# OpenDriveLab/Vista

Hardware: AMD Instinct MI355X
Metric: denoise steps/sec, 25-frame 576x1024 latent, 50-step EDM @ 1/2/4/8 GPU (higher is better)
Workload: dtype bf16; 1 GPU; 1xMI355X single GPU: 25x576x1024 (latent 25x4x72x128), 50-step EulerEDM, VanillaCFG 2.5 (N=50 images per UNet call), bf16, random-init 1.65B VideoUNet, synthetic latents; frames=25, cfg_images_per_call=50, sampler=EulerEDM s_churn=0, 50-step schedule, parallelism=single GPU

## Files before the change

include/vista_hip.h:

```cpp
#ifndef VISTA_HIP_H
#define VISTA_HIP_H
#include <stdint.h>
#ifdef __cplusplus
extern "C" {
#endif

enum { VK_AMODE_DENSE = 0, VK_AMODE_CONV3X3 = 1, VK_AMODE_TEMPORAL3 = 2, VK_AMODE_CONV3D = 3 };
enum { VK_EPI_LINEAR = 0, VK_EPI_GEGLU = 1, VK_EPI_TRANS = 2 };

typedef struct VkGemmDesc {
    const void* A;
    const void* Wt;
    void* out;
    const float* bias;
    const float* rowvec;
    const void* res1;
    const void* res2;
    int32_t M, N, K;
    int32_t lda, ldc, ld_res1, ld_res2, ldv, rows_per_vec;
    float alpha, beta;
    int32_t amode, epi, out_f32;
    int32_t H, Wd, Cin, Hout, Wout, stride, ups;
    int32_t T, S;
    int32_t tile_cfg;
// ... 205 lines not shown
```

vista_amd/csrc/gemm.hip:

```cpp
#include <stdlib.h>

#include "common.h"
#include "vista_hip.h"

#include "gemm_common.h"

extern "C" int vk_gemm_pipe_fit(const VkGemmDesc* d);
extern "C" int vk_gemm_pipe_launch(const VkGemmDesc* d, void* stream, int ksplit);
extern "C" int vk_gemm_pipe_gnstat_ok(const VkGemmDesc* d, int ksplit);
extern "C" int vk_gemm_pipe2_fit(const VkGemmDesc* d);
extern "C" int vk_gemm_pipe2_launch(const VkGemmDesc* d, void* stream);
extern "C" int vk_gemm_stream_fit(const VkGemmDesc* d);
extern "C" int vk_gemm_stream_launch(const VkGemmDesc* d, void* stream);

namespace {

constexpr int TILE5_MAX_K_DEFAULT = 320;

__device__ uint4 g_zero16;

template <int AMODE, int EPI, bool OUT_F32, int WM, int WN, int FM, int FN>
__global__ __launch_bounds__(WM * WN * 64, (WM * WN == 16) ? 4 : 2) void gemm_kernel(const VkGemmDesc p, const int ksplit) {
    constexpr int BM = WM * FM * 32, BN = WN * FN * 32;
    constexpr int NT = WM * WN * 64;
// ... 410 lines not shown
    if (full == 0 || rem == 0 || rem * 100 > (long long)max_pct * 256) return 0;
    const long long tm_main = full * 256 / tilesN;
    if (tm_main <= 0 || tm_main >= tilesM) return 0;
    const int m_split = d->m_begin + (int)tm_main * 256;
    const long long small = (long long)((d->m_end - m_split + 127) / 128) * (d->N / 160);
    if (small > 512) return 0;
    return m_split;
}

inline bool pipe2_wanted(const VkGemmDesc* d, const TileChoice& t, bool gnstat) {
    if (!(d->tile_cfg & 16) || gnstat || t.ksplit != 1 || d->amode != AMODE_DENSE || d->out_f32) return false;
    if (d->epi == EPI_LINEAR && t.cfg != 4 && t.cfg != 5 && t.cfg != 7) return false;
    return vk_gemm_pipe2_fit(d) != 0;
}

enum GemmFamily { FAM_STREAM, FAM_PIPE2, FAM_PIPE, FAM_TILED };
struct GemmPlan {
    int family;
    int cfg;
    int ksplit;
    int tail_row;
    int rowstat_slabs;
    int gnstat_slots;
};

GemmPlan plan_gemm(VkGemmDesc& d, bool rowstat, bool gnstat) {
    static const bool stream_on = [] { const char* e = getenv("VISTA_GEMM_STREAM"); return !e || atoi(e) != 0; }();
    const int force = d.tile_cfg & 7;
    if (d.m_begin == 0 && d.m_end == d.M && !(d.tile_cfg & 16) && (force == 6 || (stream_on && !rowstat))) {
        if (const int fit = vk_gemm_stream_fit(&d)) return {FAM_STREAM, 6, 1, 0, d.N / (32 * fit), 0};
    }
    if (force == 6) d.tile_cfg &= ~7;
    const TileChoice t = choose_tile(&d, rowstat, gnstat);
    GemmPlan p{FAM_TILED, t.cfg, t.ksplit, 0, 0, 0};
    if (pipe2_wanted(&d, t, gnstat)) p.family = FAM_PIPE2;
    else if (t.cfg == 7) p.family = FAM_PIPE;
    if (p.family == FAM_PIPE) p.tail_row = tail_split_row(&d, t);
    int bn, wn;
    tile_geometry(t.cfg, bn, wn);
    p.rowstat_slabs = ((d.N + bn - 1) / bn) * wn;
    if (p.family == FAM_PIPE && p.ksplit == 1 && p.tail_row == 0 && !rowstat && vk_gemm_pipe_gnstat_ok(&d, 1)) p.gnstat_slots = d.M / 64;
    return p;
}
// ... 41 lines not shown
    if (p.family == FAM_PIPE2) return vk_gemm_pipe2_launch(d, stream);
    if (p.family == FAM_PIPE && p.tail_row) {
        VkGemmDesc head = *d, tail = *d;
        head.m_end = p.tail_row;
        tail.m_begin = p.tail_row;
        rc = vk_gemm_pipe_launch(&head, stream, 1);
        return rc != VK_OK ? rc : launch_tiled(&tail, stream, 5, 1);
    }
    rc = (p.family == FAM_PIPE) ? vk_gemm_pipe_launch(d, stream, p.ksplit) : launch_tiled(d, stream, p.cfg, p.ksplit);
    if (rc != VK_OK || p.ksplit == 1) return rc;
    return launch_splitk_finish(d, stream, p.ksplit);
}

inline int validate(const VkGemmDesc* d) {
    if (!d || !d->A || !d->Wt || !d->out) return VK_EINVAL;
    if (d->M <= 0 || d->N <= 0 || d->K <= 0 || (d->K % BK) != 0 || (d->N % 4) != 0 || d->tile_cfg < 0 || (d->tile_cfg & ~(64 | 16)) > 7) return VK_EINVAL;
    if (d->m_begin < 0 || d->m_end < 0 || d->m_end > d->M || (d->m_end != 0 && d->m_begin >= d->m_end) || (d->m_end == 0 && d->m_begin >= d->M)) return VK_EINVAL;
    if ((d->m_begin != 0 || (d->m_end != 0 && d->m_end != d->M)) && d->epi == EPI_TRANS) return VK_EINVAL;
    if (d->amode != AMODE_DENSE && (d->Cin <= 0 || (d->Cin % BK) != 0)) return VK_EINVAL;
    if (d->amode == AMODE_DENSE && (d->lda % 8) != 0) return VK_EINVAL;
    if (d->amode == AMODE_CONV3X3 && (d->K != 9 * d->Cin || d->stride < 1 || d->stride > 2 || d->ups < 1 || d->ups > 2)) return VK_EINVAL;
    if (d->amode == AMODE_TEMPORAL3 && (d->K != 3 * d->Cin || d->T <= 0 || d->S <= 0)) return VK_EINVAL;
    if (d->amode == AMODE_CONV3D && (d->K != 27 * d->Cin || d->T <= 0 || d->H <= 0 || d->Wd <= 0 || d->H >= 4096 || d->Wd >= 4096 ||
                                     (long long)d->M != (long long)(d->M / (d->H * d->Wd)) * d->H * d->Wd)) return VK_EINVAL;
    if ((d->rowvec || d->rowvec2) && d->rows_per_vec <= 0) return VK_EINVAL;
    if (d->rowvec2 && (!d->res2 || d->epi != EPI_LINEAR)) return VK_EINVAL;
    if (d->A2 && (d->amode != AMODE_DENSE || d->k_split <= 0 || d->k_split >= d->K || (d->k_split % BK) != 0 || (d->lda2 % 8) != 0)) return VK_EINVAL;
    if (d->ln_stats && (d->amode != AMODE_DENSE || d->A2 || !d->ln_colsum || d->ln_parts <= 0 || d->ln_parts > 64 || !(d->ln_eps > 0.f))) return VK_EINVAL;
    if (d->rowstat_out && (d->epi != EPI_LINEAR || d->out_f32)) return VK_EINVAL;
    if (d->act != 0 && (d->act != 1 || d->epi != EPI_LINEAR)) return VK_EINVAL;
    if (d->mx8_out && (!d->mx8_scales || d->epi != EPI_LINEAR || d->out_f32 || (d->N % 320) != 0 || d->mx8_cols <= 0 || (d->mx8_cols % 320) != 0 ||
                       d->mx8_cols > d->N || (d->ld_mx8 % 16) != 0 || d->ld_mx8 < d->mx8_cols || d->ld_mx8s * 32 < d->mx8_cols ||
                       (((size_t)d->mx8_out) & 15) != 0 || d->rowstat_out || (d->ldc % 8) != 0 || (((size_t)d->out) & 15) != 0 ||
                       (d->amode != AMODE_DENSE) || d->res1 || d->res2 || d->rowvec || d->rowvec2 ||
                       (unsigned long long)d->M * 2ull * (unsigned)d->ldc >= 0xfffff000ull))
        return VK_EINVAL;
    if (d->alt_cols_from != 0 && (d->alt_cols_from < 0 || (d->alt_cols_from % 32) != 0 || d->alt_cols_from >= d->N || d->epi != EPI_LINEAR || d->out_f32 ||
                                  d->rowstat_out || d->gnstat_out || d->mx8_out))
        return VK_EINVAL;
    return VK_OK;
}

int plan_for(const VkGemmDesc* d, VkGemmDesc& q, bool rowstat, bool gnstat, GemmPlan& p) {
    const int rc = validate(d);
    if (rc != VK_OK) return rc;
    q = *d;
    norm_row_range(q);
    p = plan_gemm(q, rowstat || q.rowstat_out != nullptr, gnstat || q.gnstat_out != nullptr);
    return VK_OK;
}

}

extern "C" int vk_gemm_rowstat_parts(const VkGemmDesc* d) {
    VkGemmDesc q;
    GemmPlan p;
    const int rc = plan_for(d, q, true, false, p);
    if (rc != VK_OK) return rc;
    return (q.epi != EPI_LINEAR || q.out_f32) ? VK_EINVAL : p.rowstat_slabs;
}

extern "C" int vk_gemm_tile_choice(const VkGemmDesc* d) {
    VkGemmDesc q;
    GemmPlan p;
// ... 27 lines not shown
```

vista_amd/csrc/gemm_common.h:

```cpp
#pragma once
#include "common.h"
#include "vista_hip.h"

namespace {

enum { AMODE_DENSE = 0, AMODE_CONV3X3 = 1, AMODE_TEMPORAL3 = 2, AMODE_CONV3D = 3 };
enum { EPI_LINEAR = 0, EPI_GEGLU = 1, EPI_TRANS = 2 };

constexpr int BK = 64;

inline bool norm_row_range(VkGemmDesc& d) {
    if (d.m_end == 0) d.m_end = d.M;
    return d.m_begin >= 0 && d.m_begin < d.m_end && d.m_end <= d.M;
}


__device__ __forceinline__ uint4 widen_pair(uint2 qa, uint2 qb) {
    const auto rx = __builtin_amdgcn_permlane32_swap(qa.x, qb.x, false, false);
    const auto ry = __builtin_amdgcn_permlane32_swap(qa.y, qb.y, false, false);
    return make_uint4(rx[0], ry[0], rx[1], ry[1]);
}

#ifndef VK_EPI_NT_STORES
#define VK_EPI_NT_STORES 0
// ... 392 lines not shown
        const int c0 = 32 * fi + 8 * g + 2 * h;
        const int G0 = c0 / CPG, G1 = (c0 + 4) / CPG;
        if (G0 == G1) {
            gs[G0] = vk_dot2(w, one, gs[G0]);
            gq[G0] = vk_dot2(w, w, gq[G0]);
        } else {
            const uint32_t v0 = w & lo_mask, v1 = w & ~lo_mask;
            gs[G0] = vk_dot2(v0, one, gs[G0]);
            gq[G0] = vk_dot2(v0, v0, gq[G0]);
            gs[G1] = vk_dot2(v1, one, gs[G1]);
            gq[G1] = vk_dot2(v1, v1, gq[G1]);
        }
    }
}

template <int NRES, bool LN, bool MX, int FX, int FY, int FM, int FN, int BN, int CAP, int GNC = 0>
__device__ __forceinline__ void epilogue_linear_lds_body(const VkGemmDesc& p, f32x16_t (&acc)[FX][FY], int m0, int n0, int wm, int wn, int l31, int lh,
                                                         int stat_part, const float2* lnrow, const float* ev, int img0) {
    constexpr int MW = FM * 32, NW = FN * 32, U = FX * FY;
    constexpr int GN_NG = GNC ? NW / GNC : 1;
    constexpr int ROOM = (CAP - 16 * U - 36) / 8;
    constexpr int DA = NRES == 0 ? 0 : ((ROOM / NRES < 1 ? 1 : ROOM / NRES) < U ? (ROOM / NRES < 1 ? 1 : ROOM / NRES) : U);
    constexpr bool mx_tile = MX;
    const bool a_is_r1 = p.res1 != nullptr;
    const uint16_t* __restrict__ ra = (const uint16_t*)(a_is_r1 ? p.res1 : p.res2);
    const uint16_t* __restrict__ rb = (const uint16_t*)p.res2;
    const int lda_ = a_is_r1 ? p.ld_res1 : p.ld_res2;
    const int c0 = wn * NW + 4 * lh;
    const int wide_off = n0 + wn * NW + 8 * lh;
    bool row_ok[FY];
    int mrow[FY];
    uint32_t rao[FY], rbo[FY], oo[FY];
    char* const outb = (char*)p.out;
#pragma unroll
    for (int fj = 0; fj < FY; ++fj) {
        const int m = m0 + wm * MW + fj * 32 + l31;
        row_ok[fj] = m < p.m_end;
        mrow[fj] = row_ok[fj] ? m : p.m_end - 1;
        if (NRES >= 1) rao[fj] = ((uint32_t)mrow[fj] * (uint32_t)lda_ + (uint32_t)wide_off) * 2u;
        if (NRES == 2) rbo[fj] = ((uint32_t)mrow[fj] * (uint32_t)p.ld_res2 + (uint32_t)wide_off) * 2u;
        oo[fj] = ((uint32_t)mrow[fj] * (uint32_t)p.ldc + (uint32_t)(wide_off - (p.mx8_out ? p.mx8_cols : 0))) * 2u;
    }
    static_assert(GNC == 0 || (MW % 64 == 0 && NW == 160 && NW % GNC == 0 && !MX), "gnstat_out: wave tiles of 64-row blocks x 160 columns of whole channel groups");
    float gs[GN_NG], gq[GN_NG];
    if constexpr (GNC != 0) {
#pragma unroll
        for (int i = 0; i < GN_NG; ++i) { gs[i] = 0.f; gq[i] = 0.f; }
    }
    const uint32_t gn_lo_mask = lh ? 0u : 0xffffffffu;
    uint4 wa[U][2], wb[U][2];
    auto issue = [&](int fj, int fi, int u) {
        if (NRES >= 1) { wa[u][0] = *(const uint4*)((const char*)ra + rao[fj] + fi * 64); wa[u][1] = *(const uint4*)((const char*)ra + rao[fj] + fi * 64 + 32); }
        if (NRES == 2) { wb[u][0] = *(const uint4*)((const char*)rb + rbo[fj] + fi * 64); wb[u][1] = *(const uint4*)((const char*)rb + rbo[fj] + fi * 64 + 32); }
    };
#pragma unroll
// ... 84 lines not shown
        if constexpr (GNC != 0 && FY > 2) {
            if ((fj & 1) == 1) {
                const int mb = m0 + wm * MW + (fj >> 1) * 64;
                gn_reduce_store<GN_NG>(gs, gq, (float*)p.gnstat_out + (size_t)(mb >> 6) * 64, (n0 + wn * NW) / GNC, l31 | (lh << 5), mb < p.m_end);
#pragma unroll
                for (int i = 0; i < GN_NG; ++i) { gs[i] = 0.f; gq[i] = 0.f; }
            }
        }
    }
    if constexpr (GNC != 0 && FY == 2) {
        const int mb = m0 + wm * MW;
        gn_reduce_store<GN_NG>(gs, gq, (float*)p.gnstat_out + (size_t)(mb >> 6) * 64, (n0 + wn * NW) / GNC, l31 | (lh << 5), mb < p.m_end);
    }
}

template <int FX, int FY, int FM, int FN, int BN, int CAP = 128, int GN_CPG = 0, int GN_NRES = 0>
__device__ __forceinline__ void gemm_epilogue_linear_lds(const VkGemmDesc& p, f32x16_t (&acc)[FX][FY], int m0, int n0, int wm, int wn, int l31, int lh,
                                                         int stat_part, const float2* lnrow, const float* ev, int img0) {
    if constexpr (GN_CPG != 0) {
        epilogue_linear_lds_body<GN_NRES, false, false, FX, FY, FM, FN, BN, CAP, GN_CPG>(p, acc, m0, n0, wm, wn, l31, lh, stat_part, nullptr, ev, img0);
        return;
    }
    const int nres = (p.res1 != nullptr) + (p.res2 != nullptr);
    if constexpr (BN == 320) {
        if (p.mx8_out != nullptr && n0 < p.mx8_cols) {
            if (lnrow != nullptr) epilogue_linear_lds_body<0, true, true, FX, FY, FM, FN, BN, CAP>(p, acc, m0, n0, wm, wn, l31, lh, stat_part, lnrow, ev, img0);
            else epilogue_linear_lds_body<0, false, true, FX, FY, FM, FN, BN, CAP>(p, acc, m0, n0, wm, wn, l31, lh, stat_part, lnrow, ev, img0);
            return;
        }
    }
#define VK_EPI_BODY(NR, LNF) epilogue_linear_lds_body<NR, LNF, false, FX, FY, FM, FN, BN, CAP>(p, acc, m0, n0, wm, wn, l31, lh, stat_part, lnrow, ev, img0)
    if (lnrow != nullptr) {
        if (nres == 0) VK_EPI_BODY(0, true);
// ... 56 lines not shown
```

vista_amd/csrc/gemm_pipe.hip:

```cpp
#include "common.h"
#include "vista_hip.h"

#include "gemm_common.h"

namespace {

constexpr int PBM = 256, PBN = 320, PNT = 512;
constexpr int PFX = 5, PFY = 2;
constexpr int PRPP = PNT / 8;
constexpr int PAP = PBM / PRPP, PWP = PBN / PRPP;
constexpr int PA_BYTES = PBM * 128, PSTAGE = (PBM + PBN) * 128;
constexpr int PCAP = 256;
constexpr int APAR0 = 6 * PAP;
typedef unsigned amask_t;
constexpr unsigned P_OOB = 0xffffff00u;
constexpr unsigned long long P_LIMIT = 0xfffff000ull;
static_assert(PAP + PWP <= PFX * PFY && 8 * PAP <= 32, "the piece schedule issues one piece after each MFMA of the first k-substep");

typedef __attribute__((address_space(3))) void* lptr_t;

#define PIPE_MMA(FI, X, Y, C) C = vk_mfma(X, Y, C)

#define PIPE_SB() __builtin_amdgcn_sched_barrier(0)

template <int AMODE, int EPI, bool NT_A, bool SPLIT, int GN_CPG = 0, int GN_NRES = 0, bool PF = false>
__global__ __launch_bounds__(PNT, 2) void gemm_pipe_kernel(const VkGemmDesc p, const int ksplit) {
    static_assert(!PF || AMODE == AMODE_DENSE, "the L2 prefetch is written for the dense loader");
    constexpr int LN_OFF = 2 * PSTAGE, EV_OFF = LN_OFF + PBM * 8;
    constexpr int NTAPS = (AMODE == AMODE_CONV3X3) ? 9 : (AMODE == AMODE_TEMPORAL3) ? 3 : 1;
    constexpr bool WALK = (EPI == EPI_GEGLU);
    __shared__ __attribute__((aligned(16))) char smem[2 * PSTAGE + PBM * 8 + epi_vec_floats(PBN) * 4];
#ifdef PIPE_TIMING
    unsigned long long tm_k0, tm_dma = 0, tm_bar = 0, tm_loop = 0, tm_epi = 0, tm_ksteps = 0;
    asm volatile("s_memtime %0\n s_waitcnt lgkmcnt(0)" : "=s"(tm_k0) :: "memory");
#endif

    const int tilesN = p.N / PBN;
    const int tilesM = (p.m_end - p.m_begin + PBM - 1) / PBM;
    const int ntiles = tilesM * tilesN;
    const int tid = threadIdx.x;
    const int lane = tid & 63, wave = tid >> 6;
    const int wm = wave >> 1, wn = wave & 1;
    const int l31 = lane & 31, lh = lane >> 5;
    int kslice = 0;
    auto tile_of = [&](const int bid, int& tm, int& tn) __attribute__((always_inline)) {
        int logical = xcd_remap(bid, SPLIT ? ntiles * ksplit : ntiles);
        if (SPLIT) { kslice = logical / ntiles; logical -= kslice * ntiles; }
        if (tilesN < 8 || (long long)p.N * p.K * 2 <= (3LL << 20)) {
            tn = logical % tilesN;
            tm = logical / tilesN;
        } else {
            constexpr int GM = 8;
            const int panel = logical / (GM * tilesN), r = logical - panel * (GM * tilesN);
            const int gm = (tilesM - panel * GM < GM) ? tilesM - panel * GM : GM;
            tm = panel * GM + r % gm;
            tn = r / gm;
        }
        if constexpr (AMODE == AMODE_TEMPORAL3) {
            if (p.tile_cfg & 8) return;
            const int nblk = p.S / PBM;
            if (nblk * PBM == p.S && p.m_begin == 0 && tilesM == (p.M / p.S) * nblk && (long long)p.S * p.Cin * 2 > (3LL << 20)) {
                const int per_clip = p.T * nblk, clip = tm / per_clip, r = tm - clip * per_clip;
// ... 2 lines not shown
            }
        }
    };

    const int lc = tid & 7, lr = tid >> 3;
    const int lsrc = lc ^ ((lr >> 1) & 7);
    const int wave_u = __builtin_amdgcn_readfirstlane(wave);
    const unsigned voff_w = ((unsigned)lr * (unsigned)p.K + (unsigned)lsrc * 8u) * 2u;
    const unsigned wpass = (unsigned)PRPP * (unsigned)p.K * 2u;
    const unsigned apass = (unsigned)PRPP * (unsigned)(AMODE == AMODE_DENSE ? p.lda : p.Cin) * 2u;

    __amdgpu_buffer_rsrc_t rw, ra;
    unsigned voff_a[PAP];
    amask_t amask = 0;
    auto setup = [&](const int m0, const int n0) __attribute__((always_inline)) {
        rw = __builtin_amdgcn_make_buffer_rsrc((void*)((const uint16_t*)p.Wt + (size_t)n0 * p.K), 0, (int)((unsigned)PBN * (unsigned)p.K * 2u), 0x00020000);
        amask = 0;
        if (AMODE == AMODE_DENSE) {
            const int rows = (p.m_end - m0 < PBM) ? p.m_end - m0 : PBM;
            ra = __builtin_amdgcn_make_buffer_rsrc((void*)((const uint16_t*)p.A + (size_t)m0 * p.lda), 0,
                                                   (int)(((unsigned)(rows - 1) * (unsigned)p.lda + (unsigned)p.K) * 2u), 0x00020000);
            voff_a[0] = ((unsigned)lr * (unsigned)p.lda + (unsigned)lsrc * 8u) * 2u;
        } else if (AMODE == AMODE_CONV3X3) {
            const int hw = p.Hout * p.Wout;
            ra = __builtin_amdgcn_make_buffer_rsrc((void*)p.A, 0, (int)((unsigned)(p.M / hw) * (unsigned)(p.H * p.Wd) * (unsigned)p.Cin * 2u), 0x00020000);
#pragma unroll
            for (int i = 0; i < PAP; ++i) {
                const int m = m0 + lr + PRPP * i;
                const int img = m / hw;
                const int rem = m - img * hw;
                const int oy = rem / p.Wout, ox = rem - oy * p.Wout;
                const int y0 = oy * p.stride - (p.asym_pad ? 0 : 1), x0 = ox * p.stride - (p.asym_pad ? 0 : 1);
                const int sh = p.ups - 1;
// ... 37 lines not shown
            const unsigned v = voff_a[0] + (unsigned)j * apass;
            if (NT_A) __builtin_amdgcn_raw_ptr_buffer_load_lds(ra, dst, 16, v, (unsigned)kb, 0, 2);
            else __builtin_amdgcn_raw_ptr_buffer_load_lds(ra, dst, 16, v, (unsigned)kb, 0, 0);
        } else if (AMODE == AMODE_CONV3X3) {
            const int ky = tap / 3, kx = tap - ky * 3;
            const bool ok = ((amask >> (6 * j + ky)) & (amask >> (6 * j + 3 + kx)) & 1u) != 0;
            unsigned v;
            if (p.ups == 2) {
                const unsigned dy = ((unsigned)((amask >> (APAR0 + 2 * j)) & 1u) + (unsigned)(ky + 1)) >> 1, dx = ((unsigned)((amask >> (APAR0 + 1 + 2 * j)) & 1u) + (unsigned)(kx + 1)) >> 1;
                v = voff_a[j] + (dy * (unsigned)p.Wd + dx) * ((unsigned)p.Cin * 2u);
            } else {
                v = voff_a[j] + (unsigned)((ky * p.Wd + kx) * p.Cin) * 2u;
            }
            if (!ok) v = P_OOB;
            __builtin_amdgcn_raw_ptr_buffer_load_lds(ra, dst, 16, v, (unsigned)c0b, 0, 0);
        } else {
            const unsigned tapoff = (unsigned)((tap - 1) * p.S * p.Cin) * 2u;
            const bool ok = ((amask >> (3 * j + tap)) & 1u) != 0;
            const unsigned v = ok ? voff_a[0] + (unsigned)j * apass + tapoff : P_OOB;
            __builtin_amdgcn_raw_ptr_buffer_load_lds(ra, dst, 16, v, (unsigned)c0b, 0, 0);
        }
    };
    auto dma_next = [&]() __attribute__((always_inline)) {
        kb += BK * 2;
        if (AMODE != AMODE_DENSE) {
            if (++tap == NTAPS) { tap = 0; c0b += BK * 2; }
        }
    };
    auto dma_q = [&](const int q, const int stage) __attribute__((always_inline)) { dma_piece(q < PAP ? PWP + q : q - PAP, stage); };

// ... 165 lines not shown

        int te = tid;
        asm volatile("" : "+v"(te));
        const int e_wave = te >> 6, e_l31 = te & 31, e_lh = (te >> 5) & 1;
        const int e_wm = e_wave >> 1, e_wn = e_wave & 1;
        const float2* const lnp = p.ln_stats != nullptr ? lnrow : nullptr;
        if constexpr (SPLIT) {
            VkGemmDesc q = p;
            q.out = (float*)p.splitk_ws + (size_t)kslice * p.M * p.N;
            q.ldc = p.N;
            q.bias = nullptr; q.rowvec = nullptr; q.res1 = nullptr; q.res2 = nullptr;
            q.alpha = 1.f; q.beta = 0.f;
            q.rowvec2 = nullptr; q.ln_stats = nullptr; q.rowstat_out = nullptr; q.act = 0;
            gemm_epilogue<EPI_LINEAR, true, PFX, PFY, PFY, 5>(q, acc, m0, n0, e_wm, e_wn, e_l31, e_lh);
        } else if constexpr (EPI == EPI_GEGLU) gemm_epilogue_geglu_lds<PFX, PFY, PFY, 5, PBN>(p, acc, m0, n0, e_wm, e_wn, e_l31, e_lh, lnp, epi_vec);
        else gemm_epilogue_linear_lds<PFX, PFY, PFY, 5, PBN, PCAP, GN_CPG, GN_NRES>(p, acc, m0, n0, e_wm, e_wn, e_l31, e_lh, tn * 2 + e_wn, lnp, epi_vec, eplan.img0);
#ifdef PIPE_TIMING
        unsigned long long tm_t2;
        asm volatile("s_memtime %0\n s_waitcnt lgkmcnt(0)" : "=s"(tm_t2) :: "memory");
        tm_epi += tm_t2 - tm_t1;
#endif
        if (!more) break;
        __syncthreads();
        bid = nbid; tm = ntm; tn = ntn;
        m0 = p.m_begin + tm * PBM; n0 = tn * PBN;
        eplan = plan_of(m0);
        stage_tile_vectors(m0, n0, eplan);
        __syncthreads();
        st ^= 1;
    }
    if constexpr (PF) asm volatile("" :: "v"(pf_dummy));
// ... 36 lines not shown
    }
    if constexpr (AMODE == AMODE_DENSE) {
        if (ntiles <= 256 && d->K >= 3 * BK && (d->lda % 64) == 0 && (((size_t)d->A) & 127) == 0) {
            if (nt_a) hipLaunchKernelGGL((gemm_pipe_kernel<AMODE, EPI, true, false, 0, 0, true>), dim3(grid), dim3(PNT), 0, stream, *d, 1);
            else hipLaunchKernelGGL((gemm_pipe_kernel<AMODE, EPI, false, false, 0, 0, true>), dim3(grid), dim3(PNT), 0, stream, *d, 1);
            VK_CHECK_LAUNCH();
            return VK_OK;
        }
    }
    if (nt_a) hipLaunchKernelGGL((gemm_pipe_kernel<AMODE, EPI, AMODE == AMODE_DENSE, false>), dim3(grid), dim3(PNT), 0, stream, *d, 1);
    else hipLaunchKernelGGL((gemm_pipe_kernel<AMODE, EPI, false, false>), dim3(grid), dim3(PNT), 0, stream, *d, 1);
    VK_CHECK_LAUNCH();
    return VK_OK;
}

}

extern "C" int vk_gemm_pipe_fit(const VkGemmDesc* d) {
    if ((d->epi != EPI_LINEAR && d->epi != EPI_GEGLU) || d->out_f32 || (d->N % PBN) != 0 || d->mx8_out || d->A2) return 0;
    if (d->epi == EPI_GEGLU && d->amode != AMODE_DENSE) return 0;
    if (!epi_fast_everywhere(*d, d->epi, PBM)) return 0;
    if ((unsigned long long)PBN * d->K * 2ull >= P_LIMIT) return 0;
    if (d->amode == AMODE_DENSE) return ((unsigned long long)PBM * d->lda * 2ull < P_LIMIT) ? 1 : 0;
    if (d->amode == AMODE_CONV3X3) {
        if (d->ups == 2 && (d->stride != 1 || d->asym_pad)) return 0;
        const long long hw = (long long)d->Hout * d->Wout;
        if (hw <= 0 || (d->M % hw) != 0) return 0;
        return ((unsigned long long)(d->M / hw) * d->H * d->Wd * d->Cin * 2ull < P_LIMIT) ? 1 : 0;
    }
    if (d->amode == AMODE_TEMPORAL3) {
        if (d->halo_prev || d->halo_next) return 0;
        return ((unsigned long long)d->M * d->Cin * 2ull < P_LIMIT) ? 1 : 0;
    }
// ... 1 lines not shown
}

extern "C" int vk_gemm_pipe_gnstat_ok(const VkGemmDesc* d, int ksplit) {
    if (!vk_gemm_pipe_fit(d) || ksplit != 1 || d->epi != EPI_LINEAR || d->out_f32) return 0;
    if (d->amode != AMODE_CONV3X3 && d->amode != AMODE_TEMPORAL3) return 0;
    if (d->N != 320 && d->N != 640 && d->N != 1280) return 0;
    if (d->ln_stats || d->mx8_out || d->act || d->rowstat_out || (d->res1 && d->res2)) return 0;
    if (d->gn_rows <= 0 || (d->gn_rows % 64) != 0 || (d->M % d->gn_rows) != 0) return 0;
    if (d->m_begin != 0 || (d->m_end != 0 && d->m_end != d->M)) return 0;
    return 1;
}

extern "C" int vk_gemm_pipe_launch(const VkGemmDesc* d, void* stream_, int ksplit) {
    hipStream_t stream = (hipStream_t)stream_;
    if (!vk_gemm_pipe_fit(d)) return VK_EINVAL;
    if (ksplit > 1 && (d->epi != EPI_LINEAR || !d->splitk_ws || d->ln_stats || d->rowstat_out || d->act)) return VK_EINVAL;
    if (d->gnstat_out && !vk_gemm_pipe_gnstat_ok(d, ksplit)) return VK_EINVAL;
    if (d->amode == AMODE_DENSE) return d->epi == EPI_GEGLU ? pipe_launch<AMODE_DENSE, EPI_GEGLU>(d, stream, ksplit) : pipe_launch<AMODE_DENSE, EPI_LINEAR>(d, stream, ksplit);
    if (d->amode == AMODE_CONV3X3) return pipe_launch<AMODE_CONV3X3, EPI_LINEAR>(d, stream, ksplit);
    if (d->amode == AMODE_TEMPORAL3) return pipe_launch<AMODE_TEMPORAL3, EPI_LINEAR>(d, stream, ksplit);
    return VK_EINVAL;
}
```

vista_amd/modules/diffusionmodules/openaimodel.py:

```python
from typing import Iterable

import torch.nn as nn

from ... import ops
from ..attention import FP8, Packable
from .util import Dropout, SiLU, conv_nd, linear, normalization, timestep_embedding, zero_module


class TimestepBlock(nn.Module):
    """Any module where forward() takes timestep embeddings as a second argument."""


class TimestepEmbedSequential(nn.Sequential, TimestepBlock):

    def forward(self, x, emb_silu, context=None, frame_idx=None, num_frames=None, H=None, W=None, shard=None, full=None):
        from ..video_attention import SpatialVideoTransformer
        from .video_model import VideoResBlock
        layers = list(self)
        x_gn = None
        for i, layer in enumerate(layers):
            if isinstance(layer, VideoResBlock):
                x_gn = ops.GnPartials() if i + 1 < len(layers) and isinstance(layers[i + 1], SpatialVideoTransformer) else None
                x = layer(x, emb_silu, num_frames, H, W, shard=shard, full=full, out_gn=x_gn)
            elif isinstance(layer, SpatialVideoTransformer):
# ... 4 lines not shown
            else:
                raise TypeError(f"unexpected layer {type(layer).__name__} in TimestepEmbedSequential")
        return x, H, W


class Upsample(nn.Module, Packable):
    def __init__(self, channels, use_conv, dims=2, out_channels=None, padding=1, third_up=False, kernel_size=3, scale_factor=2):
        super().__init__()
        if dims != 2 or not use_conv or kernel_size != 3 or scale_factor != 2 or padding != 1:
            raise NotImplementedError("Vista uses Upsample(dims=2, use_conv=True, k=3, x2)")
        self.channels = channels
        self.out_channels = out_channels or channels
        self.use_conv, self.dims = use_conv, dims
        self.conv = conv_nd(dims, self.channels, self.out_channels, kernel_size, padding=padding)

    def _pack(self, dev):
        return ops.pack_conv3x3(self.conv.weight, self.conv.bias, device=dev)

    def forward(self, x, H, W):
        assert x.shape[-1] == self.channels
        out, Ho, Wo = ops.conv3x3(x, self.packed(), x.shape[0], H, W, ups=2)
        return out, Ho, Wo


class Downsample(nn.Module, Packable):
    def __init__(self, channels, use_conv, dims=2, out_channels=None, padding=1, third_down=False):
        super().__init__()
        if dims != 2 or not use_conv or padding != 1:
            raise NotImplementedError("Vista uses Downsample(dims=2, use_conv=True)")
        self.channels = channels
        self.out_channels = out_channels or channels
        self.use_conv, self.dims = use_conv, dims
        self.op = conv_nd(dims, self.channels, self.out_channels, 3, stride=2, padding=padding)

    def _pack(self, dev):
        return ops.pack_conv3x3(self.op.weight, self.op.bias, device=dev)
# ... 124 lines not shown
```

vista_amd/ops.py:

```python
import ctypes as C
import math
import os
import threading

import torch

from . import _lib
from ._lib import VkFp8Args, VkGemmDesc, check

AMODE_DENSE, AMODE_CONV3X3, AMODE_TEMPORAL3, AMODE_CONV3D = 0, 1, 2, 3
EPI_LINEAR, EPI_GEGLU, EPI_TRANS = 0, 1, 2
ACT = torch.float16 if _lib.ACT_DTYPE == "fp16" else torch.bfloat16
BF16 = ACT
F32 = torch.float32


class storage:

    def __init__(self, dtype):
        if dtype not in (torch.bfloat16, torch.float16):
            raise ValueError("ops.storage: torch.bfloat16 or torch.float16")
        self.dtype, self.name = dtype, ("fp16" if dtype is torch.float16 else "bf16")

    def __enter__(self):
        global ACT, BF16
# ... 39 lines not shown
def _rows2d(t, name):
    if t.stride(-1) != 1:
        raise ValueError(f"{name}: last dim must be contiguous")
    t2 = t.reshape(-1, t.shape[-1]) if t.is_contiguous() else t
    if t2.dim() != 2:
        raise ValueError(f"{name}: pass a 2-D strided view")
    return t2, t2.stride(0)


def ceil_to(x, m):
    return (x + m - 1) // m * m


class PackedWeight:

    __slots__ = ("wt", "bias", "N", "K", "geglu", "colsum", "ln_eps", "ffout")

    def __init__(self, wt, bias, N, K, geglu=False, colsum=None, ln_eps=0.0, ffout=False):
        self.wt, self.bias, self.N, self.K, self.geglu, self.colsum, self.ln_eps = wt, bias, N, K, geglu, colsum, ln_eps
        self.ffout = ffout


def _finish_pack(w2d, bias, device, geglu=False, ln=None):
    N, K = w2d.shape
    Kp = ceil_to(K, 64)
    Np = max(ceil_to(N, 256), ceil_to(N, 320))
    colsum, eps = None, 0.0
    if ln is not None:
        gamma, beta, eps = ln
        if Kp != K:
            raise ValueError("LayerNorm fold needs K % 64 == 0")
        gamma, beta = gamma.detach().float().to(w2d.device), beta.detach().float().to(w2d.device)
        t = w2d @ beta
        bias = t if bias is None else bias.to(w2d.device) + t
        w2d = w2d * gamma[None, :]
# ... 58 lines not shown
    return _finish_pack(w[perm], b[perm], device, geglu=True, ln=None if ln is None else _ln_tuple(ln))


def _slab_major(w):
    cout, taps, cin = w.shape
    return w.reshape(cout, taps, cin // 64, 64).permute(0, 2, 1, 3).reshape(cout, taps * cin)


def pack_conv3x3(weight, bias=None, cin_pad=None, device="cuda"):
    w = weight.detach().float().permute(0, 2, 3, 1).contiguous()
    cout, _, _, cin = w.shape
    cp = cin_pad or ceil_to(cin, 64)
    if cp != cin:
        w = torch.nn.functional.pad(w, (0, cp - cin))
    return _finish_pack(_slab_major(w.reshape(cout, 9, cp)), None if bias is None else bias.detach().float(), device)


def pack_conv_t3(weight, bias=None, device="cuda", cin_pad=None):
    w = weight.detach().float()[:, :, :, 0, 0].permute(0, 2, 1).contiguous()
    cout, _, cin = w.shape
    if cin_pad and cin_pad != cin:
        w = torch.nn.functional.pad(w, (0, cin_pad - cin))
        cin = cin_pad
    if cin % 64:
        raise ValueError("temporal conv needs Cin % 64 == 0")
    return _finish_pack(_slab_major(w), None if bias is None else bias.detach().float(), device)


TILE_CFG = 0

# ... 285 lines not shown
    pad = 1 if asym_pad else 2
    Hout = (He + pad - 3) // stride + 1
    Wout = (We + pad - 3) // stride + 1
    M = n_img * Hout * Wout
    if out is None:
        out = torch.empty((M, pw.N), dtype=F32 if out_f32 else BF16, device=x.device)
    d = VkGemmDesc()
    d.A, d.lda = _p(x), cin
    d.amode, d.epi = AMODE_CONV3X3, EPI_LINEAR
    d.H, d.Wd, d.Cin, d.Hout, d.Wout, d.stride, d.ups = H, W, cin, Hout, Wout, stride, ups
    d.asym_pad = 1 if asym_pad else 0
    _fill_epilogue(d, pw, out, M, rowvec, Hout * Wout, res1, res2, alpha, beta)
    _ask_gn(d, gn, Hout * Wout, x.device)
    _gemm(d)
    return (out.view(n_img, Hout * Wout, pw.N) if out.is_contiguous() else out), Hout, Wout


def conv_t3(x, pw, T, S, *, out=None, out_f32=False, rowvec=None, res1=None, res2=None, alpha=1.0, beta=0.0, halo_prev=None,
            halo_next=None, gn=None):
    _need(x, BF16, "x")
    if not x.is_contiguous():
        raise ValueError("conv_t3: x must be contiguous")
    cin = x.shape[-1]
    if pw.K != 3 * cin:
        raise ValueError("conv_t3: weight K mismatch")
    M = x.shape[0] * x.shape[1]
    if out is None:
        out = torch.empty((M, pw.N), dtype=F32 if out_f32 else BF16, device=x.device)
    d = VkGemmDesc()
    d.A, d.lda = _p(x), cin
# ... 799 lines not shown
```

Before: 6.264 steps/s.

## Fold nearest-upsample 3x3 conv into four 2x2 sub-pixel convolutions

Adds an UPCONV2X2 A-mode to the pipelined GEMM. The 2x nearest-upsample followed by a 3x3 conv is computed as four phase classes, each a 2x2 conv on the low-resolution input with pre-summed weights. The epilogue scatters each class's outputs to their interleaved positions. This cuts the reduction length from 9*Cin to 4*Cin and avoids reading the upsampled input, at the cost of a new loader/epilogue path, a second weight pack, and a fallback to the 3x3 path when the new kernel does not fit.

```diff
diff --git a/include/vista_hip.h b/include/vista_hip.h
--- a/include/vista_hip.h
+++ b/include/vista_hip.h
@@ -5,7 +5,7 @@
 extern "C" {
 #endif
 
-enum { VK_AMODE_DENSE = 0, VK_AMODE_CONV3X3 = 1, VK_AMODE_TEMPORAL3 = 2, VK_AMODE_CONV3D = 3 };
+enum { VK_AMODE_DENSE = 0, VK_AMODE_CONV3X3 = 1, VK_AMODE_TEMPORAL3 = 2, VK_AMODE_CONV3D = 3, VK_AMODE_UPCONV2X2 = 4 };
 enum { VK_EPI_LINEAR = 0, VK_EPI_GEGLU = 1, VK_EPI_TRANS = 2 };
 
 typedef struct VkGemmDesc {
diff --git a/vista_amd/csrc/gemm.hip b/vista_amd/csrc/gemm.hip
--- a/vista_amd/csrc/gemm.hip
+++ b/vista_amd/csrc/gemm.hip
@@ -448,7 +448,7 @@
     return vk_gemm_pipe2_fit(d) != 0;
 }
 
-enum GemmFamily { FAM_STREAM, FAM_PIPE2, FAM_PIPE, FAM_TILED };
+enum GemmFamily { FAM_NONE = -1, FAM_STREAM, FAM_PIPE2, FAM_PIPE, FAM_TILED };
 struct GemmPlan {
     int family;
     int cfg;
@@ -461,6 +461,15 @@
 GemmPlan plan_gemm(VkGemmDesc& d, bool rowstat, bool gnstat) {
     static const bool stream_on = [] { const char* e = getenv("VISTA_GEMM_STREAM"); return !e || atoi(e) != 0; }();
     const int force = d.tile_cfg & 7;
+    if (d.amode == AMODE_UPCONV2X2) {
+        VkGemmDesc nine = d;
+        nine.amode = AMODE_CONV3X3;
+        nine.K = 9 * d.Cin;
+        nine.tile_cfg &= ~8;
+        const TileChoice t = choose_tile(&nine, false, false);
+        const bool ok = t.cfg == 7 && t.ksplit == 1 && !rowstat && !gnstat && vk_gemm_pipe_fit(&d);
+        return {ok ? FAM_PIPE : FAM_NONE, 7, 1, 0, 0, 0};
+    }
     if (d.m_begin == 0 && d.m_end == d.M && !(d.tile_cfg & 16) && (force == 6 || (stream_on && !rowstat))) {
         if (const int fit = vk_gemm_stream_fit(&d)) return {FAM_STREAM, 6, 1, 0, d.N / (32 * fit), 0};
     }
@@ -532,13 +541,25 @@
 
 inline int validate(const VkGemmDesc* d) {
     if (!d || !d->A || !d->Wt || !d->out) return VK_EINVAL;
-    if (d->M <= 0 || d->N <= 0 || d->K <= 0 || (d->K % BK) != 0 || (d->N % 4) != 0 || d->tile_cfg < 0 || (d->tile_cfg & ~(64 | 16)) > 7) return VK_EINVAL;
+    const int upc_bits = d->amode == AMODE_UPCONV2X2 ? 8 : 0;
+    if (d->M <= 0 || d->N <= 0 || d->K <= 0 || (d->K % BK) != 0 || (d->N % 4) != 0 || d->tile_cfg < 0 || (d->tile_cfg & ~(64 | 16 | upc_bits)) > 7) return VK_EINVAL;
+    if (d->amode < AMODE_DENSE || d->amode > AMODE_UPCONV2X2) return VK_EINVAL;
     if (d->m_begin < 0 || d->m_end < 0 || d->m_end > d->M || (d->m_end != 0 && d->m_begin >= d->m_end) || (d->m_end == 0 && d->m_begin >= d->M)) return VK_EINVAL;
     if ((d->m_begin != 0 || (d->m_end != 0 && d->m_end != d->M)) && d->epi == EPI_TRANS) return VK_EINVAL;
     if (d->amode != AMODE_DENSE && (d->Cin <= 0 || (d->Cin % BK) != 0)) return VK_EINVAL;
     if (d->amode == AMODE_DENSE && (d->lda % 8) != 0) return VK_EINVAL;
     if (d->amode == AMODE_CONV3X3 && (d->K != 9 * d->Cin || d->stride < 1 || d->stride > 2 || d->ups < 1 || d->ups > 2)) return VK_EINVAL;
     if (d->amode == AMODE_TEMPORAL3 && (d->K != 3 * d->Cin || d->T <= 0 || d->S <= 0)) return VK_EINVAL;
+    if (d->amode == AMODE_UPCONV2X2) {
+        if (d->K != 4 * d->Cin || d->ups != 2 || d->stride != 1 || d->asym_pad || d->H <= 0 || d->Wd <= 0 || d->Hout != 2 * d->H || d->Wout != 2 * d->Wd) return VK_EINVAL;
+        const long long hw4 = 4ll * d->H * d->Wd;
+        if ((d->M % hw4) != 0 || (d->rowvec && d->rows_per_vec != hw4)) return VK_EINVAL;
+        if (d->epi != EPI_LINEAR || d->out_f32 || d->res1 || d->res2 || d->rowvec2 || d->gnstat_out || d->rowstat_out || d->mx8_out || d->ln_stats || d->A2 ||
+            d->halo_prev || d->halo_next || d->act || d->alt_cols_from)
+            return VK_EINVAL;
+        if (d->m_begin != 0 || (d->m_end != 0 && d->m_end != d->M)) return VK_EINVAL;
+        if ((d->tile_cfg & (64 | 16)) != 0 || ((d->tile_cfg & 7) != 0 && (d->tile_cfg & 7) != 7)) return VK_EINVAL;
+    }
     if (d->amode == AMODE_CONV3D && (d->K != 27 * d->Cin || d->T <= 0 || d->H <= 0 || d->Wd <= 0 || d->H >= 4096 || d->Wd >= 4096 ||
                                      (long long)d->M != (long long)(d->M / (d->H * d->Wd)) * d->H * d->Wd)) return VK_EINVAL;
     if ((d->rowvec || d->rowvec2) && d->rows_per_vec <= 0) return VK_EINVAL;
@@ -565,7 +586,7 @@
     q = *d;
     norm_row_range(q);
     p = plan_gemm(q, rowstat || q.rowstat_out != nullptr, gnstat || q.gnstat_out != nullptr);
-    return VK_OK;
+    return p.family == FAM_NONE ? VK_EINVAL : VK_OK;
 }
 
 }
diff --git a/vista_amd/csrc/gemm_common.h b/vista_amd/csrc/gemm_common.h
--- a/vista_amd/csrc/gemm_common.h
+++ b/vista_amd/csrc/gemm_common.h
@@ -4,7 +4,7 @@
 
 namespace {
 
-enum { AMODE_DENSE = 0, AMODE_CONV3X3 = 1, AMODE_TEMPORAL3 = 2, AMODE_CONV3D = 3 };
+enum { AMODE_DENSE = 0, AMODE_CONV3X3 = 1, AMODE_TEMPORAL3 = 2, AMODE_CONV3D = 3, AMODE_UPCONV2X2 = 4 };
 enum { EPI_LINEAR = 0, EPI_GEGLU = 1, EPI_TRANS = 2 };
 
 constexpr int BK = 64;
@@ -430,9 +430,9 @@
     }
 }
 
-template <int NRES, bool LN, bool MX, int FX, int FY, int FM, int FN, int BN, int CAP, int GNC = 0>
+template <int NRES, bool LN, bool MX, int FX, int FY, int FM, int FN, int BN, int CAP, int GNC = 0, bool UPC = false>
 __device__ __forceinline__ void epilogue_linear_lds_body(const VkGemmDesc& p, f32x16_t (&acc)[FX][FY], int m0, int n0, int wm, int wn, int l31, int lh,
-                                                         int stat_part, const float2* lnrow, const float* ev, int img0) {
+                                                         int stat_part, const float2* lnrow, const float* ev, int img0, int cls = 0) {
     constexpr int MW = FM * 32, NW = FN * 32, U = FX * FY;
     constexpr int GN_NG = GNC ? NW / GNC : 1;
     constexpr int ROOM = (CAP - 16 * U - 36) / 8;
@@ -455,6 +455,11 @@
         mrow[fj] = row_ok[fj] ? m : p.m_end - 1;
         if (NRES >= 1) rao[fj] = ((uint32_t)mrow[fj] * (uint32_t)lda_ + (uint32_t)wide_off) * 2u;
         if (NRES == 2) rbo[fj] = ((uint32_t)mrow[fj] * (uint32_t)p.ld_res2 + (uint32_t)wide_off) * 2u;
+        if constexpr (UPC) {
+            const int hw = p.H * p.Wd, img = mrow[fj] / hw, rem = mrow[fj] - img * hw, sy = rem / p.Wd, sx = rem - sy * p.Wd;
+            const uint32_t orow = (uint32_t)(img * 4 * hw + (2 * sy + (cls >> 1)) * 2 * p.Wd + 2 * sx + (cls & 1));
+            oo[fj] = (orow * (uint32_t)p.ldc + (uint32_t)wide_off) * 2u;
+        } else
         oo[fj] = ((uint32_t)mrow[fj] * (uint32_t)p.ldc + (uint32_t)(wide_off - (p.mx8_out ? p.mx8_cols : 0))) * 2u;
     }
     static_assert(GNC == 0 || (MW % 64 == 0 && NW == 160 && NW % GNC == 0 && !MX), "gnstat_out: wave tiles of 64-row blocks x 160 columns of whole channel groups");
@@ -569,9 +574,13 @@
     }
 }
 
-template <int FX, int FY, int FM, int FN, int BN, int CAP = 128, int GN_CPG = 0, int GN_NRES = 0>
+template <int FX, int FY, int FM, int FN, int BN, int CAP = 128, int GN_CPG = 0, int GN_NRES = 0, bool UPC = false>
 __device__ __forceinline__ void gemm_epilogue_linear_lds(const VkGemmDesc& p, f32x16_t (&acc)[FX][FY], int m0, int n0, int wm, int wn, int l31, int lh,
-                                                         int stat_part, const float2* lnrow, const float* ev, int img0) {
+                                                         int stat_part, const float2* lnrow, const float* ev, int img0, int cls = 0) {
+    if constexpr (UPC) {
+        epilogue_linear_lds_body<0, false, false, FX, FY, FM, FN, BN, CAP, 0, true>(p, acc, m0, n0, wm, wn, l31, lh, stat_part, nullptr, ev, img0, cls);
+        return;
+    }
     if constexpr (GN_CPG != 0) {
         epilogue_linear_lds_body<GN_NRES, false, false, FX, FY, FM, FN, BN, CAP, GN_CPG>(p, acc, m0, n0, wm, wn, l31, lh, stat_part, nullptr, ev, img0);
         return;
diff --git a/vista_amd/csrc/gemm_pipe.hip b/vista_amd/csrc/gemm_pipe.hip
--- a/vista_amd/csrc/gemm_pipe.hip
+++ b/vista_amd/csrc/gemm_pipe.hip
@@ -27,7 +27,9 @@
 __global__ __launch_bounds__(PNT, 2) void gemm_pipe_kernel(const VkGemmDesc p, const int ksplit) {
     static_assert(!PF || AMODE == AMODE_DENSE, "the L2 prefetch is written for the dense loader");
     constexpr int LN_OFF = 2 * PSTAGE, EV_OFF = LN_OFF + PBM * 8;
-    constexpr int NTAPS = (AMODE == AMODE_CONV3X3) ? 9 : (AMODE == AMODE_TEMPORAL3) ? 3 : 1;
+    constexpr int NTAPS = (AMODE == AMODE_CONV3X3) ? 9 : (AMODE == AMODE_TEMPORAL3) ? 3 : (AMODE == AMODE_UPCONV2X2) ? 4 : 1;
+    constexpr bool UPC = (AMODE == AMODE_UPCONV2X2);
+    static_assert(!UPC || (EPI == EPI_LINEAR && !SPLIT && GN_CPG == 0), "the folded upsample convolution: plain LINEAR epilogue, one launch");
     constexpr bool WALK = (EPI == EPI_GEGLU);
     __shared__ __attribute__((aligned(16))) char smem[2 * PSTAGE + PBM * 8 + epi_vec_floats(PBN) * 4];
 #ifdef PIPE_TIMING
@@ -43,9 +45,14 @@
     const int wm = wave >> 1, wn = wave & 1;
     const int l31 = lane & 31, lh = lane >> 5;
     int kslice = 0;
+    int cls = 0;
     auto tile_of = [&](const int bid, int& tm, int& tn) __attribute__((always_inline)) {
-        int logical = xcd_remap(bid, SPLIT ? ntiles * ksplit : ntiles);
+        int logical = xcd_remap(bid, SPLIT ? ntiles * ksplit : UPC ? ntiles * 4 : ntiles);
         if (SPLIT) { kslice = logical / ntiles; logical -= kslice * ntiles; }
+        if (UPC) {
+            if (p.tile_cfg & 8) { cls = logical & 3; logical >>= 2; }
+            else { cls = logical / ntiles; logical -= cls * ntiles; }
+        }
         if (tilesN < 8 || (long long)p.N * p.K * 2 <= (3LL << 20)) {
             tn = logical % tilesN;
             tm = logical / tilesN;
@@ -78,9 +85,29 @@
     unsigned voff_a[PAP];
     amask_t amask = 0;
     auto setup = [&](const int m0, const int n0) __attribute__((always_inline)) {
-        rw = __builtin_amdgcn_make_buffer_rsrc((void*)((const uint16_t*)p.Wt + (size_t)n0 * p.K), 0, (int)((unsigned)PBN * (unsigned)p.K * 2u), 0x00020000);
+        const size_t wrow0 = UPC ? (size_t)cls * (size_t)((p.N + 255) / 256 * 256) + (size_t)n0 : (size_t)n0;
+        rw = __builtin_amdgcn_make_buffer_rsrc((void*)((const uint16_t*)p.Wt + wrow0 * p.K), 0, (int)((unsigned)PBN * (unsigned)p.K * 2u), 0x00020000);
         amask = 0;
-        if (AMODE == AMODE_DENSE) {
+        if (AMODE == AMODE_UPCONV2X2) {
+            const int hw = p.H * p.Wd;
+            ra = __builtin_amdgcn_make_buffer_rsrc((void*)p.A, 0, (int)((unsigned)p.M * (unsigned)p.Cin * 2u), 0x00020000);
+#pragma unroll
+            for (int i = 0; i < PAP; ++i) {
+                const int m = m0 + lr + PRPP * i;
+                const int img = m / hw;
+                const int rem = m - img * hw;
+                const int sy = rem / p.Wd, sx = rem - sy * p.Wd;
+                const int y0 = sy + (cls >> 1) - 1, x0 = sx + (cls & 1) - 1;
+                voff_a[i] = ((unsigned)((img * p.H + y0) * p.Wd + x0) * (unsigned)p.Cin + (unsigned)lsrc * 8u) * 2u;
+                unsigned mk = 0;
+#pragma unroll
+                for (int t = 0; t < 2; ++t) {
+                    if (m < p.m_end && y0 + t >= 0 && y0 + t < p.H) mk |= 1u << t;
+                    if (x0 + t >= 0 && x0 + t < p.Wd) mk |= 4u << t;
+                }
+                amask |= (amask_t)mk << (4 * i);
+            }
+        } else if (AMODE == AMODE_DENSE) {
             const int rows = (p.m_end - m0 < PBM) ? p.m_end - m0 : PBM;
             ra = __builtin_amdgcn_make_buffer_rsrc((void*)((const uint16_t*)p.A + (size_t)m0 * p.lda), 0,
                                                    (int)(((unsigned)(rows - 1) * (unsigned)p.lda + (unsigned)p.K) * 2u), 0x00020000);
@@ -148,6 +175,11 @@
             }
             if (!ok) v = P_OOB;
             __builtin_amdgcn_raw_ptr_buffer_load_lds(ra, dst, 16, v, (unsigned)c0b, 0, 0);
+        } else if (AMODE == AMODE_UPCONV2X2) {
+            const int dy = tap >> 1, dx = tap & 1;
+            const bool ok = ((amask >> (4 * j + dy)) & (amask >> (4 * j + 2 + dx)) & 1u) != 0;
+            const unsigned v = ok ? voff_a[j] + (unsigned)((dy * p.Wd + dx) * p.Cin) * 2u : P_OOB;
+            __builtin_amdgcn_raw_ptr_buffer_load_lds(ra, dst, 16, v, (unsigned)c0b, 0, 0);
         } else {
             const unsigned tapoff = (unsigned)((tap - 1) * p.S * p.Cin) * 2u;
             const bool ok = ((amask >> (3 * j + tap)) & 1u) != 0;
@@ -343,7 +375,7 @@
             q.rowvec2 = nullptr; q.ln_stats = nullptr; q.rowstat_out = nullptr; q.act = 0;
             gemm_epilogue<EPI_LINEAR, true, PFX, PFY, PFY, 5>(q, acc, m0, n0, e_wm, e_wn, e_l31, e_lh);
         } else if constexpr (EPI == EPI_GEGLU) gemm_epilogue_geglu_lds<PFX, PFY, PFY, 5, PBN>(p, acc, m0, n0, e_wm, e_wn, e_l31, e_lh, lnp, epi_vec);
-        else gemm_epilogue_linear_lds<PFX, PFY, PFY, 5, PBN, PCAP, GN_CPG, GN_NRES>(p, acc, m0, n0, e_wm, e_wn, e_l31, e_lh, tn * 2 + e_wn, lnp, epi_vec, eplan.img0);
+        else gemm_epilogue_linear_lds<PFX, PFY, PFY, 5, PBN, PCAP, GN_CPG, GN_NRES, UPC>(p, acc, m0, n0, e_wm, e_wn, e_l31, e_lh, tn * 2 + e_wn, lnp, epi_vec, eplan.img0, cls);
 #ifdef PIPE_TIMING
         unsigned long long tm_t2;
         asm volatile("s_memtime %0\n s_waitcnt lgkmcnt(0)" : "=s"(tm_t2) :: "memory");
@@ -410,9 +442,39 @@
     return VK_OK;
 }
 
+inline VkGemmDesc upconv_class_desc(const VkGemmDesc* d) {
+    VkGemmDesc q = *d;
+    q.M = d->M / 4;
+    q.m_begin = 0;
+    q.m_end = q.M;
+    q.rows_per_vec = d->H * d->Wd;
+    return q;
+}
+
+int upconv_fit(const VkGemmDesc* d) {
+    if (d->epi != EPI_LINEAR || d->out_f32 || (d->N % PBN) != 0 || d->mx8_out || d->A2 || d->res1 || d->res2 || d->rowvec2 || d->gnstat_out || d->rowstat_out ||
+        d->ln_stats || d->act || d->alt_cols_from || d->halo_prev || d->halo_next)
+        return 0;
+    if (d->m_begin != 0 || (d->m_end != 0 && d->m_end != d->M)) return 0;
+    VkGemmDesc q = *d;
+    q.rows_per_vec = d->H * d->Wd;
+    if (!epi_fast_everywhere(q, EPI_LINEAR, PBM)) return 0;
+    if ((unsigned long long)PBN * d->K * 2ull >= P_LIMIT) return 0;
+    return ((unsigned long long)(d->M / 4) * d->Cin * 2ull < P_LIMIT) ? 1 : 0;
+}
+
+int upconv_launch(const VkGemmDesc* d, hipStream_t stream) {
+    const VkGemmDesc q = upconv_class_desc(d);
+    const int tilesN = q.N / PBN, tilesM = (q.M + PBM - 1) / PBM;
+    hipLaunchKernelGGL((gemm_pipe_kernel<AMODE_UPCONV2X2, EPI_LINEAR, false, false>), dim3(4 * tilesM * tilesN), dim3(PNT), 0, stream, q, 1);
+    VK_CHECK_LAUNCH();
+    return VK_OK;
+}
+
 }
 
 extern "C" int vk_gemm_pipe_fit(const VkGemmDesc* d) {
+    if (d->amode == AMODE_UPCONV2X2) return upconv_fit(d);
     if ((d->epi != EPI_LINEAR && d->epi != EPI_GEGLU) || d->out_f32 || (d->N % PBN) != 0 || d->mx8_out || d->A2) return 0;
     if (d->epi == EPI_GEGLU && d->amode != AMODE_DENSE) return 0;
     if (!epi_fast_everywhere(*d, d->epi, PBM)) return 0;
@@ -444,6 +506,7 @@
 extern "C" int vk_gemm_pipe_launch(const VkGemmDesc* d, void* stream_, int ksplit) {
     hipStream_t stream = (hipStream_t)stream_;
     if (!vk_gemm_pipe_fit(d)) return VK_EINVAL;
+    if (d->amode == AMODE_UPCONV2X2) return ksplit == 1 ? upconv_launch(d, stream) : VK_EINVAL;
     if (ksplit > 1 && (d->epi != EPI_LINEAR || !d->splitk_ws || d->ln_stats || d->rowstat_out || d->act)) return VK_EINVAL;
     if (d->gnstat_out && !vk_gemm_pipe_gnstat_ok(d, ksplit)) return VK_EINVAL;
     if (d->amode == AMODE_DENSE) return d->epi == EPI_GEGLU ? pipe_launch<AMODE_DENSE, EPI_GEGLU>(d, stream, ksplit) : pipe_launch<AMODE_DENSE, EPI_LINEAR>(d, stream, ksplit);
diff --git a/vista_amd/modules/diffusionmodules/openaimodel.py b/vista_amd/modules/diffusionmodules/openaimodel.py
--- a/vista_amd/modules/diffusionmodules/openaimodel.py
+++ b/vista_amd/modules/diffusionmodules/openaimodel.py
@@ -1,3 +1,4 @@
+import os
 from typing import Iterable
 
 import torch.nn as nn
@@ -42,12 +43,23 @@
         self.use_conv, self.dims = use_conv, dims
         self.conv = conv_nd(dims, self.channels, self.out_channels, kernel_size, padding=padding)
 
+    _nine = None
+
     def _pack(self, dev):
+        if os.environ.get("VISTA_UPCONV_FOLD", "1") != "0" and self.channels % 64 == 0:
+            return ops.pack_upconv2x2(self.conv.weight, self.conv.bias, device=dev)
         return ops.pack_conv3x3(self.conv.weight, self.conv.bias, device=dev)
 
     def forward(self, x, H, W):
         assert x.shape[-1] == self.channels
-        out, Ho, Wo = ops.conv3x3(x, self.packed(), x.shape[0], H, W, ups=2)
+        pw = self.packed()
+        if pw.classes == 4:
+            if ops.upconv2x2_fits(x, pw, x.shape[0], H, W):
+                return ops.upconv2x2(x, pw, x.shape[0], H, W)
+            if self._nine is None or self._nine[1] is not pw:
+                object.__setattr__(self, "_nine", (ops.pack_conv3x3(self.conv.weight, self.conv.bias, device=x.device), pw))
+            pw = self._nine[0]
+        out, Ho, Wo = ops.conv3x3(x, pw, x.shape[0], H, W, ups=2)
         return out, Ho, Wo
 
 
diff --git a/vista_amd/ops.py b/vista_amd/ops.py
--- a/vista_amd/ops.py
+++ b/vista_amd/ops.py
@@ -8,7 +8,7 @@
 from . import _lib
 from ._lib import VkFp8Args, VkGemmDesc, check
 
-AMODE_DENSE, AMODE_CONV3X3, AMODE_TEMPORAL3, AMODE_CONV3D = 0, 1, 2, 3
+AMODE_DENSE, AMODE_CONV3X3, AMODE_TEMPORAL3, AMODE_CONV3D, AMODE_UPCONV2X2 = 0, 1, 2, 3, 4
 EPI_LINEAR, EPI_GEGLU, EPI_TRANS = 0, 1, 2
 ACT = torch.float16 if _lib.ACT_DTYPE == "fp16" else torch.bfloat16
 BF16 = ACT
@@ -78,11 +78,12 @@
 
 class PackedWeight:
 
-    __slots__ = ("wt", "bias", "N", "K", "geglu", "colsum", "ln_eps", "ffout")
-
-    def __init__(self, wt, bias, N, K, geglu=False, colsum=None, ln_eps=0.0, ffout=False):
+    __slots__ = ("wt", "bias", "N", "K", "geglu", "colsum", "ln_eps", "ffout", "classes")
+
+    def __init__(self, wt, bias, N, K, geglu=False, colsum=None, ln_eps=0.0, ffout=False, classes=1):
         self.wt, self.bias, self.N, self.K, self.geglu, self.colsum, self.ln_eps = wt, bias, N, K, geglu, colsum, ln_eps
         self.ffout = ffout
+        self.classes = classes
 
 
 def _finish_pack(w2d, bias, device, geglu=False, ln=None):
@@ -171,6 +172,40 @@
     if cp != cin:
         w = torch.nn.functional.pad(w, (0, cp - cin))
     return _finish_pack(_slab_major(w.reshape(cout, 9, cp)), None if bias is None else bias.detach().float(), device)
+
+
+UPCONV_ROWS = (((0,), (1, 2)), ((0, 1), (2,)))
+
+
+def fold_upconv2x2(weight):
+    w = weight.detach()
+    classes = []
+    for a in (0, 1):
+        rows = [sum(w[:, :, ky] for ky in UPCONV_ROWS[a][dy]) for dy in (0, 1)]
+        for b in (0, 1):
+            classes.append(torch.stack([torch.stack([sum(r[:, :, kx] for kx in UPCONV_ROWS[b][dx]) for dx in (0, 1)], -1) for r in rows], -2))
+    return torch.stack(classes)
+
+
+def pack_upconv2x2(weight, bias=None, device="cuda"):
+    w = fold_upconv2x2(weight.detach().float())
+    _, cout, cin = w.shape[:3]
+    if cin % 64:
+        raise ValueError("pack_upconv2x2 needs Cin % 64 == 0")
+    Np = max(ceil_to(cout, 256), ceil_to(cout, 320))
+    wt = torch.zeros((4 * Np, 4 * cin), dtype=BF16, device=device)
+    for c in range(4):
+        wt[c * Np:c * Np + cout] = _slab_major(w[c].permute(0, 2, 3, 1).reshape(cout, 4, cin)).to(device=device, dtype=BF16)
+    b = None
+    if bias is not None:
+        b = torch.zeros((Np,), dtype=F32, device=device)
+        b[:cout] = bias.detach().to(device=device, dtype=F32)
+    return PackedWeight(wt, b, ceil_to(cout, 4), 4 * cin, classes=4)
+
+
+def unpack_upconv2x2(pw, cout):
+    Np, cin = pw.wt.shape[0] // 4, pw.K // 4
+    return pw.wt.view(4, Np, cin // 64, 2, 2, 64)[:, :cout].permute(0, 1, 2, 5, 3, 4).reshape(4, cout, cin, 2, 2)
 
 
 def pack_conv_t3(weight, bias=None, device="cuda", cin_pad=None):
@@ -486,6 +521,45 @@
     _ask_gn(d, gn, Hout * Wout, x.device)
     _gemm(d)
     return (out.view(n_img, Hout * Wout, pw.N) if out.is_contiguous() else out), Hout, Wout
+
+
+UPCONV_CLASS_FASTEST = int(os.environ.get("VISTA_UPCONV_ORDER", "0")) != 0
+
+
+def _upconv_desc(x, pw, n_img, H, W, rowvec, out):
+    cin = x.shape[-1]
+    d = VkGemmDesc()
+    d.A, d.lda = _p(x), cin
+    d.amode, d.epi = AMODE_UPCONV2X2, EPI_LINEAR
+    d.H, d.Wd, d.Cin, d.Hout, d.Wout, d.stride, d.ups = H, W, cin, 2 * H, 2 * W, 1, 2
+    _fill_epilogue(d, pw, out, n_img * 4 * H * W, rowvec, 4 * H * W, None, None, 1.0, 0.0)
+    stream = _prepare(d)
+    if UPCONV_CLASS_FASTEST:
+        d.tile_cfg |= 8
+    return d, stream
+
+
+def upconv2x2_fits(x, pw, n_img, H, W, rowvec=None, out=None):
+    if out is None:
+        out = x
+    d, _ = _upconv_desc(x, pw, n_img, H, W, rowvec, out)
+    d.ldc = pw.N
+    return _lib.load().vk_gemm_tile_choice(C.byref(d)) > 0
+
+
+def upconv2x2(x, pw, n_img, H, W, rowvec=None, out=None):
+    _need(x, BF16, "x")
+    if not x.is_contiguous():
+        raise ValueError("upconv2x2: x must be contiguous")
+    cin = x.shape[-1]
+    if pw.classes != 4 or pw.K != 4 * cin:
+        raise ValueError(f"upconv2x2: needs a pack_upconv2x2 weight with K = 4*{cin}")
+    M = n_img * 4 * H * W
+    if out is None:
+        out = torch.empty((M, pw.N), dtype=BF16, device=x.device)
+    d, stream = _upconv_desc(x, pw, n_img, H, W, rowvec, out)
+    check(_lib.load().vk_gemm_bf16(C.byref(d), stream), "vk_gemm_bf16 (folded upsample convolution)")
+    return (out.view(n_img, 4 * H * W, pw.N) if out.is_contiguous() else out), 2 * H, 2 * W
 
 
 def conv_t3(x, pw, T, S, *, out=None, out_f32=False, rowvec=None, res1=None, res2=None, alpha=1.0, beta=0.0, halo_prev=None,
```

After: 6.385 steps/s (median of 6 runs). 1.02x the previous value.
